# alibaba/EasyRec

Hardware: AMD Instinct MI355X
Metric: global examples/sec + emb HBM GB/s, DeepFM Criteo-shape b4096 @1/2/4/8 GPU (higher is better)
Workload: dtype f32; 1 GPU; DeepFM synthetic Criteo: deepfm_criteo.config (39 features: 26 hashed x 1000000 rows + 13 projected, D=16 deep + D=1 wide, batch 4096 per GPU, optimizer adam_optimizer (lazy dense decay, closed-form replay), ids zipf, hipGraph replay); timed steps cycle over 256 distinct device-generated batches after 1024 untimed pre-conditioning steps; global_batch=4096, parallelism=single GPU

## Files before the change

### easyrec_amd/csrc/er_embedding.hip

```cpp
#include <algorithm>
#include <cmath>
#include <cstring>
#include <vector>

#include "er_common.h"
#include "er_gemm_core.h"
#include "er_dense_tail.h"
#include "er_decay.h"
#include "er_grad_finish.h"

namespace er {

constexpr uint32_t kInvalidKey = 0xFFFFFFFFu;

__host__ __device__ __forceinline__ void lane_geom(int dim, int& V, int& G) {
  V = (dim % 4 == 0) ? 4 : 1;
  const int n = dim / V;
  G = 1;
  while (G < n) G <<= 1;
}

__device__ __forceinline__ int find_lookup(const int32_t* __restrict__ blk_start, int n, int bid) {
  int lo = 0, hi = n;
  while (hi - lo > 1) {
// ... 1457 lines not shown
  while (i + 1 < ma.n && static_cast<int>(blockIdx.x) >= ma.start[i + 1]) ++i;
  const RunArgs& a = ma.a[i];
  const int bid = blockIdx.x - ma.start[i];
  if (a.V == 4)
    tile_body<4>(bid, smem, a.skeys, a.svals, a.ent_gptr, a.ent_scale, a.n, a.dim, a.G, a.tab, ma.opt_kind, ma.hyper, a.ro,
                 a.tile_first, a.tile_last);
  else
    tile_body<1>(bid, smem, a.skeys, a.svals, a.ent_gptr, a.ent_scale, a.n, a.dim, a.G, a.tab, ma.opt_kind, ma.hyper, a.ro,
                 a.tile_first, a.tile_last);
}

__device__ __forceinline__ void tile_multi_block(int b, const RunMulti& ma, float* smem) {
  int i = 0;
  while (i + 1 < ma.n && b >= ma.start[i + 1]) ++i;
  const RunArgs& a = ma.a[i];
  const int bid = b - ma.start[i];
  if (a.V == 4)
    tile_body<4>(bid, smem, a.skeys, a.svals, a.ent_gptr, a.ent_scale, a.n, a.dim, a.G, a.tab, ma.opt_kind, ma.hyper, a.ro,
                 a.tile_first, a.tile_last);
  else
    tile_body<1>(bid, smem, a.skeys, a.svals, a.ent_gptr, a.ent_scale, a.n, a.dim, a.G, a.tab, ma.opt_kind, ma.hyper, a.ro,
                 a.tile_first, a.tile_last);
}

__global__ void __launch_bounds__(kBlock)
emb_reduce_local_wgrad_kernel(RunMulti ma, GroupedArgs ga, int n_gemm, int n_tile, LossTailArgs lt) {
  extern __shared__ __attribute__((aligned(16))) float smem[];
  const int bid = blockIdx.x;
  if (bid < n_gemm) {
    const GroupedCoords c = grouped_coords(ga, bid);
    if (c.split < 0) return;
    gemm_f32_block<false, false>(ga.p[c.p], c.tile, c.split, smem, c.plain);
    return;
  }
  if (bid - n_gemm < n_tile) tile_multi_block(bid - n_gemm, ma, smem);
  else loss_tail_body<kBlock>(lt, smem);
}

__device__ __forceinline__ void fix_block(int b, const RunMulti& ma) {
  int i = 0;
  while (i + 1 < ma.n && b >= ma.start[i + 1]) ++i;
  const RunArgs& a = ma.a[i];
  const int bid = b - ma.start[i];
  if (a.V == 4)
    fix_body<4>(bid, a.skeys, a.n, a.dim, a.G, a.T, a.n_tiles, a.tab, ma.opt_kind, ma.hyper, a.ro, a.tile_first,
                a.tile_last, a.aux);
  else
    fix_body<1>(bid, a.skeys, a.n, a.dim, a.G, a.T, a.n_tiles, a.tab, ma.opt_kind, ma.hyper, a.ro, a.tile_first,
                a.tile_last, a.aux);
}

__global__ void __launch_bounds__(kBlock)
emb_bwd_fix_multi_kernel(RunMulti ma) {
  fix_block(blockIdx.x, ma);
}

__global__ void __launch_bounds__(kBlock)
emb_bwd_fix_reduce_kernel(RunMulti ma, GroupedReduceArgs ra, int n_fix) {
  const int b = blockIdx.x;
  if (b < n_fix) fix_block(b, ma);
  else splitk_reduce_grouped_block<4>(ra, b - n_fix);
}

__global__ void __launch_bounds__(kBlock)
emb_bwd_fix_opt_kernel(RunMulti ma, GroupedReduceArgs ra, DenseOptArgs da, int n_fix) {
  __shared__ float red[4];
  const int b = blockIdx.x;
  if (b < n_fix) fix_block(b, ma);
  else dense_opt_block(da, ra, b - n_fix, red);
}

constexpr int kSegSortMax = 8192;
constexpr int kSegSortMin = 256;

template <typename C>
__device__ __forceinline__ void seg_cmpx(C& a, C& b, bool up) {
  const bool sw = (a > b) == up;
  const C lo = sw ? b : a, hi = sw ? a : b;
  a = lo;
  b = hi;
}

constexpr int kRadixBits = 5;
template <int E>
__device__ __forceinline__ void seg_radix_sort_narrow(uint32_t (&x)[E], uint32_t* buf , int P, int logP, uint32_t rel_max) {
  constexpr int NB = 1 << kRadixBits;
  constexpr int kMaxWaves = kSegSortMax / 8 / 64;
  __shared__ uint32_t cnt[NB * kMaxWaves];
  __shared__ uint32_t wtot[kMaxWaves];
  const int t = threadIdx.x, lane = t & 63, wave = t >> 6, nW = static_cast<int>(blockDim.x >> 6);
  const int n_cnt = NB * nW;
  uint32_t* A = buf;
  uint32_t* B = buf + P;
#pragma unroll
  for (int e = 0; e < E; ++e) A[t * E + e] = x[e];
  __syncthreads();
  const int key_bits = 32 - __clz(static_cast<int>(rel_max | 1u));
  const int chunk = wave * 64 * E;
  const unsigned long long lt_mask = (1ull << lane) - 1ull;
  uint32_t key[E];
#pragma unroll
  for (int e = 0; e < E; ++e) key[e] = A[chunk + e * 64 + lane];
  for (int shift = logP; shift < logP + key_bits; shift += kRadixBits) {
    if (t < n_cnt) cnt[t] = 0u;
    __syncthreads();
    uint32_t rank[E], slot[E];
#pragma unroll
    for (int e = 0; e < E; ++e) {
      const uint32_t d = (key[e] >> shift) & static_cast<uint32_t>(NB - 1);
      unsigned long long m = ~0ull;
#pragma unroll
      for (int b = 0; b < kRadixBits; ++b) {
        const bool bit = ((d >> b) & 1u) != 0u;
        const unsigned long long bal = __ballot(bit);
        m &= bit ? bal : ~bal;
      }
      const uint32_t lower = static_cast<uint32_t>(__popcll(m & lt_mask));
      const int sl = static_cast<int>(d) * nW + wave;
      const uint32_t prior = cnt[sl];
      rank[e] = prior + lower;
      slot[e] = static_cast<uint32_t>(sl);
      if (lower == 0u) cnt[sl] = prior + static_cast<uint32_t>(__popcll(m));
    }
    __syncthreads();
    uint32_t v = 0u, inc = 0u;
    if (t < n_cnt) v = cnt[t];
    inc = v;
#pragma unroll
    for (int dd = 1; dd < 64; dd <<= 1) {
      const uint32_t o = __shfl_up(inc, dd, 64);
      if (lane >= dd) inc += o;
    }
    if (lane == 63) wtot[wave] = inc;
    __syncthreads();
    uint32_t before = 0u;
    for (int w = 0; w < wave; ++w) before += wtot[w];
    if (t < n_cnt) cnt[t] = before + inc - v;
    __syncthreads();
#pragma unroll
    for (int e = 0; e < E; ++e) B[cnt[slot[e]] + rank[e]] = key[e];
    __syncthreads();
    uint32_t* T = A; A = B; B = T;
#pragma unroll
    for (int e = 0; e < E; ++e) key[e] = A[chunk + e * 64 + lane];
  }
#pragma unroll
  for (int e = 0; e < E; ++e) x[e] = A[t * E + e];
}

template <int E, bool HEADS, bool NARROW, bool INLINE>
__device__ __forceinline__ void seg_sort_body(int lk, const uint32_t* __restrict__ keys_in, const int64_t* __restrict__ ent_base,
                        const er_lookup_desc* __restrict__ descs, int P, Route rt, uint32_t* __restrict__ keys_out,
                        uint32_t* __restrict__ vals_out, uint32_t* __restrict__ flags_out,
                        uint32_t* __restrict__ hidx_out, uint32_t* __restrict__ seg_count, int skip_one_row,
                        unsigned long long* sk_raw, uint32_t* __restrict__ ukeys_seg = nullptr,
                        int64_t n_limit = INT64_MAX) {
  typedef typename std::conditional<NARROW, uint32_t, unsigned long long>::type C;
  C* sk = reinterpret_cast<C*>(sk_raw);
  constexpr int L = E == 8 ? 3 : (E == 4 ? 2 : 1);
  static_assert(E == 2 || E == 4 || E == 8, "E");
  const int t = threadIdx.x;
  const int i0 = t * E;
  const int64_t base = ent_base[lk];
  const int64_t end = ent_base[lk + 1] < n_limit ? ent_base[lk + 1] : n_limit;
  const int cnt = end > base ? static_cast<int>(end - base) : 0;
  const int logP = __ffs(P) - 1;
  const bool routed = rt.local_base != nullptr;
  const uint32_t stride = static_cast<uint32_t>(rt.shard_stride);
  uint32_t key_base = 0u, rows = 0u, srows = 1u;
  if (NARROW) {
    const er_lookup_desc& d = descs[lk];
    if (routed) {
      srows = static_cast<uint32_t>((d.rows + rt.world - 1) / rt.world);
      rows = srows * static_cast<uint32_t>(rt.world);
      key_base = static_cast<uint32_t>(rt.local_base[lk]);
    } else {
      rows = static_cast<uint32_t>(d.rows);
      key_base = static_cast<uint32_t>(d.key_base);
    }
  }
  auto key_of = [&](C c) -> uint32_t {
    if (NARROW) {
      const uint32_t rel = static_cast<uint32_t>(c >> logP);
      if (rel >= rows) return kInvalidKey;
      if (!routed) return rel + key_base;
      const uint32_t owner = rel / srows;
      return owner * stride + key_base + (rel - owner * srows);
    }
    return static_cast<uint32_t>(static_cast<unsigned long long>(c) >> 32);
  };
  C x[E];
#pragma unroll
  for (int e = 0; e < E; ++e) {
    const int i = i0 + e;
    if (i >= cnt) {
      x[e] = static_cast<C>(~0ull);
    } else if (INLINE) {
      const er_lookup_desc& d = descs[lk];
      const int64_t id = d.ids[i];
      bool ok = !(id < 0 || id >= d.rows);
      if (d.weights != nullptr && d.combiner != ER_COMBINER_SUM && !(d.weights[i] > 0.f)) ok = false;
      if (skip_one_row && d.rows == 1) ok = false;
      if (NARROW) {
        const uint32_t rel = ok ? static_cast<uint32_t>(id) : static_cast<uint32_t>(d.rows);
        x[e] = static_cast<C>((rel << logP) | static_cast<uint32_t>(i));
      } else {
        const uint32_t key = ok ? static_cast<uint32_t>(d.key_base + id) : kInvalidKey;
        x[e] = static_cast<C>((static_cast<unsigned long long>(key) << 32) | static_cast<unsigned>(base + i));
      }
    } else if (NARROW) {
      const uint32_t key = keys_in[base + i];
      uint32_t rel = rows;
      if (key != kInvalidKey) {
        if (routed) {
          const uint32_t owner = key / stride;
          rel = owner * srows + (key - owner * stride - key_base);
        } else {
          rel = key - key_base;
        }
      }
      x[e] = static_cast<C>((rel << logP) | static_cast<uint32_t>(i));
    } else {
      x[e] = static_cast<C>((static_cast<unsigned long long>(keys_in[base + i]) << 32) | static_cast<unsigned>(base + i));
    }
  }
  if constexpr (NARROW) {
    seg_radix_sort_narrow<E>(x, reinterpret_cast<uint32_t*>(sk_raw), P, logP, rows);
  } else
  for (int k = 2; k <= P; k <<= 1) {
    int j = k >> 1;
    bool in_lds = false;
    while (j >= 64 * E) {
      if (!in_lds) {
#pragma unroll
        for (int e = 0; e < E; ++e) sk[i0 + e] = x[e];
        __syncthreads();
      }
      const int b = __ffs(j) - 1, lb = b - L + 1;
      const int bs = ((t >> lb) << (b + 1)) | (t & ((1 << lb) - 1));
      const bool up = (bs & k) == 0;
      C y[E];
#pragma unroll
      for (int c = 0; c < E; ++c) y[c] = sk[bs + (c << lb)];
#pragma unroll
      for (int jj = E / 2; jj > 0; jj >>= 1)
#pragma unroll
        for (int c = 0; c < E; ++c)
          if ((c & jj) == 0) seg_cmpx(y[c], y[c | jj], up);
#pragma unroll
      for (int c = 0; c < E; ++c) sk[bs + (c << lb)] = y[c];
      __syncthreads();
      in_lds = true;
      j >>= L;
    }
    if (in_lds) {
#pragma unroll
      for (int e = 0; e < E; ++e) x[e] = sk[i0 + e];
    }
    if (j >= E) {
      const bool up = (i0 & k) == 0;
      for (; j >= E; j >>= 1) {
        const int lj = j / E;
        const bool keep_min = ((t & lj) == 0) == up;
#pragma unroll
        for (int e = 0; e < E; ++e) {
          const C o = __shfl_xor(x[e], lj);
          const C mn = x[e] < o ? x[e] : o, mx = x[e] < o ? o : x[e];
          x[e] = keep_min ? mn : mx;
        }
      }
    }
#pragma unroll
    for (int jj = E / 2; jj > 0; jj >>= 1) {
      if (jj <= j) {
#pragma unroll
        for (int e = 0; e < E; ++e)
          if ((e & jj) == 0) seg_cmpx(x[e], x[e | jj], ((i0 + e) & k) == 0);
      }
    }
  }
  uint32_t kk[E], ow[E];
#pragma unroll
  for (int e = 0; e < E; ++e) {
    kk[e] = key_of(x[e]);
    ow[e] = routed ? kk[e] / stride : 0u;
  }
#pragma unroll
  for (int e = 0; e < E; ++e) {
    const int i = i0 + e;
    if (i < cnt) {
      keys_out[base + i] = kk[e];
      vals_out[base + i] = NARROW ? static_cast<uint32_t>(base) + (static_cast<uint32_t>(x[e]) & static_cast<uint32_t>(P - 1))
                                  : static_cast<uint32_t>(static_cast<unsigned long long>(x[e]) & 0xFFFFFFFFu);
    }
  }
  if (HEADS) {
    __shared__ uint32_t wave_sum[kSegSortMax / 8 / 64];
    uint32_t* k32 = reinterpret_cast<uint32_t*>(sk_raw);
    __syncthreads();
#pragma unroll
    for (int e = 0; e < E; ++e) k32[i0 + e] = kk[e];
    __syncthreads();
    uint32_t prev = i0 > 0 ? k32[i0 - 1] : kInvalidKey;
    uint32_t f[E], c = 0;
#pragma unroll
    for (int e = 0; e < E; ++e) {
      const uint32_t key = kk[e];
      f[e] = (key != kInvalidKey && (i0 + e == 0 || prev != key)) ? 1u : 0u;
      c += f[e];
      prev = key;
    }
    const int lane = t & 63, wave = t >> 6, n_waves = blockDim.x >> 6;
    uint32_t inc = c;
#pragma unroll
    for (int d = 1; d < 64; d <<= 1) {
      const uint32_t o = __shfl_up(inc, d, 64);
      if (lane >= d) inc += o;
    }
    if (lane == 63) wave_sum[wave] = inc;
    __syncthreads();
    uint32_t before = 0, total = 0;
    for (int w = 0; w < n_waves; ++w) {
      const uint32_t ws = wave_sum[w];
      if (w < wave) before += ws;
      total += ws;
    }
    uint32_t run = before + inc - c;
#pragma unroll
    for (int e = 0; e < E; ++e) {
      const int i = i0 + e;
      if (i < cnt) {
        flags_out[base + i] = f[e];
        hidx_out[base + i] = run;
        if (ukeys_seg != nullptr && f[e]) ukeys_seg[base + run] = kk[e];
      }
      run += f[e];
    }
    if (!routed) {
      if (t == 0) seg_count[lk] = total;
    } else {
      __shared__ uint32_t owner_cnt[64];
      if (t < 64) owner_cnt[t] = 0u;
      __syncthreads();
#pragma unroll
      for (int e = 0; e < E; ++e)
        if (f[e]) atomicAdd(&owner_cnt[ow[e]], 1u);
      __syncthreads();
      if (t < 64) seg_count[lk * 64 + t] = owner_cnt[t];
    }
  }
}

template <int E, bool HEADS, bool NARROW>
__global__ void __launch_bounds__(kSegSortMax / 8)
emb_segment_sort_kernel(const uint32_t* __restrict__ keys_in, const int64_t* __restrict__ ent_base,
                        const er_lookup_desc* __restrict__ descs, int P, Route rt, uint32_t* __restrict__ keys_out,
                        uint32_t* __restrict__ vals_out, uint32_t* __restrict__ flags_out,
                        uint32_t* __restrict__ hidx_out, uint32_t* __restrict__ seg_count) {
  extern __shared__ __attribute__((aligned(16))) unsigned long long sk_raw[];
  seg_sort_body<E, HEADS, NARROW, false>(blockIdx.x, keys_in, ent_base, descs, P, rt, keys_out, vals_out, flags_out, hidx_out,
                                         seg_count, 0, sk_raw);
}

template <int E, bool NARROW>
__global__ void __launch_bounds__(kSegSortMax / 8)
emb_front_sort_kernel(const int64_t* __restrict__ ent_base, const er_lookup_desc* __restrict__ descs, int n_lookups, int P,
                      uint32_t* __restrict__ keys_out, uint32_t* __restrict__ vals_out, uint32_t* __restrict__ flags_out,
                      uint32_t* __restrict__ hidx_out, uint32_t* __restrict__ seg_count, int skip_one_row, DecayTabDev tabs,
                      const float* __restrict__ hist, const int64_t* __restrict__ counter, uint32_t* __restrict__ ukeys_seg) {
  extern __shared__ __attribute__((aligned(16))) unsigned long long sk_raw[];
  if (static_cast<int>(blockIdx.x) >= n_lookups) {
    const int k = (static_cast<int>(blockIdx.x) - n_lookups) * static_cast<int>(blockDim.x >> 6) + static_cast<int>(threadIdx.x >> 6) + 1;
    if (k > tabs.K) return;
    const int64_t s_end = *counter - 1;
    const float mine = decay_sum_wave(tabs, hist, s_end - 1 - k, k);
    const int lane = threadIdx.x & 63;
    float* A = tabs.A + static_cast<int64_t>(kDecayKMax) * kDecayLd;
    if (lane < kDecayLd) A[static_cast<int64_t>(k - 1) * kDecayLd + lane] = mine;
    return;
  }
  seg_sort_body<E, true, NARROW, true>(blockIdx.x, nullptr, ent_base, descs, P, Route{1, 0, nullptr}, keys_out, vals_out,
                                       flags_out, hidx_out, seg_count, skip_one_row, sk_raw, ukeys_seg);
}

template <int E, bool NARROW>
__global__ void __launch_bounds__(kSegSortMax / 8)
emb_front_fwd_kernel(const int64_t* __restrict__ ent_base, const er_lookup_desc* __restrict__ descs, int n_lookups, int P,
                     uint32_t* __restrict__ keys_out, uint32_t* __restrict__ vals_out, uint32_t* __restrict__ flags_out,
                     uint32_t* __restrict__ hidx_out, uint32_t* __restrict__ seg_count, int skip_one_row,
                     uint32_t* __restrict__ ukeys_seg, const er_lookup_desc* __restrict__ fwd_descs,
                     const int32_t* __restrict__ fwd_blk_start, int fwd_lookups, int fwd_blocks,
                     float* __restrict__ sumsq_partials, FwdLazy lz) {
  extern __shared__ __attribute__((aligned(16))) unsigned long long sk_raw[];
  if (static_cast<int>(blockIdx.x) < n_lookups) {
    seg_sort_body<E, true, NARROW, true>(blockIdx.x, nullptr, ent_base, descs, P, Route{1, 0, nullptr}, keys_out, vals_out,
                                         flags_out, hidx_out, seg_count, skip_one_row, sk_raw, ukeys_seg);
    return;
  }
  __shared__ float red[kSegSortMax / 8 / 64];
  const int per_wg = static_cast<int>(blockDim.x) / kBlock;
  const int vb = (static_cast<int>(blockIdx.x) - n_lookups) * per_wg + static_cast<int>(threadIdx.x) / kBlock;
  const int vt = static_cast<int>(threadIdx.x) % kBlock;
  float ss = 0.f;
  if (vb < fwd_blocks) ss = fwd_rows<true>(vb, vt, fwd_descs, fwd_blk_start, fwd_lookups, &lz);
  if (sumsq_partials) {
    ss = wave_sum(ss);
    const int wid = threadIdx.x >> 6;
    if ((threadIdx.x & 63) == 0) red[wid] = ss;
    __syncthreads();
    if (vt == 0 && vb < fwd_blocks) {
      const int w0 = (static_cast<int>(threadIdx.x) / kBlock) * 4;
      sumsq_partials[vb] = (red[w0] + red[w0 + 1]) + (red[w0 + 2] + red[w0 + 3]);
    }
  }
}

template <int E>
__global__ void __launch_bounds__(kSegSortMax / 8)
emb_chunk_sort_kernel(const uint32_t* __restrict__ keys_in, const int64_t* __restrict__ chunk_base, int P, int64_t n,
                      uint32_t* __restrict__ keys_out, uint32_t* __restrict__ vals_out) {
  extern __shared__ __attribute__((aligned(16))) unsigned long long sk_raw[];
  seg_sort_body<E, false, false, false>(blockIdx.x, keys_in, chunk_base, nullptr, P, Route{1, 0, nullptr}, keys_out, vals_out,
                                        nullptr, nullptr, nullptr, 0, sk_raw, nullptr, n);
}

constexpr int kChunkSortMax = 4096;
constexpr int kMergeVt = 8;
constexpr int kMergeTile = kBlock * kMergeVt;

__device__ __forceinline__ unsigned long long merge_comp(const uint32_t* __restrict__ k, const uint32_t* __restrict__ v, int64_t i) {
  return (static_cast<unsigned long long>(k[i]) << 32) | v[i];
}

template <typename GetA, typename GetB>
__device__ __forceinline__ int merge_path(int d, int na, int nb, GetA a_at, GetB b_at) {
  int lo = d > nb ? d - nb : 0, hi = d < na ? d : na;
  while (lo < hi) {
    const int mid = (lo + hi) >> 1;
    if (a_at(mid) < b_at(d - 1 - mid)) lo = mid + 1; else hi = mid;
  }
  return lo;
}

__global__ void __launch_bounds__(kBlock)
emb_merge_pass_kernel(const uint32_t* __restrict__ kin, const uint32_t* __restrict__ vin, int64_t n, int64_t run,
                      uint32_t* __restrict__ kout, uint32_t* __restrict__ vout) {
  __shared__ unsigned long long sm[kMergeTile];
  __shared__ int s_lo[2], s_hi[2];
  const int tid = threadIdx.x;
  const int64_t o0 = static_cast<int64_t>(blockIdx.x) * kMergeTile;
  const int64_t o1 = o0 + kMergeTile < n ? o0 + kMergeTile : n;
  const int64_t pair0 = (o0 / (2 * run)) * (2 * run);
  const int64_t a_beg = pair0;
  const int64_t a_end = a_beg + run < n ? a_beg + run : n;
  const int64_t b_end = a_end + run < n ? a_end + run : n;
  const int na = static_cast<int>(a_end - a_beg), nb = static_cast<int>(b_end - a_end);
  {
    constexpr int K = kBlock / 2;
    const int half = tid / K, t = tid % K;
    const int d = static_cast<int>((half == 0 ? o0 : o1) - pair0);
    if (t == 0) {
      s_lo[half] = d > nb ? d - nb : 0;
      s_hi[half] = d < na ? d : na;
    }
    __syncthreads();
    for (;;) {
      const int lo = s_lo[half], hi = s_hi[half];
      const int r = hi - lo;
      if (!__syncthreads_or(r > 0)) break;
      if (r > 0) {
        const int p = lo + static_cast<int>((static_cast<int64_t>(r) * (t + 1)) / (K + 1));
        const bool below = merge_comp(kin, vin, a_beg + p) < merge_comp(kin, vin, a_end + (d - 1 - p));
        if (below) atomicMax(&s_lo[half], p + 1); else atomicMin(&s_hi[half], p);
      }
      __syncthreads();
    }
  }
  const int a0 = s_lo[0], a1 = s_lo[1];
  const int b0 = static_cast<int>(o0 - pair0) - a0, b1 = static_cast<int>(o1 - pair0) - a1;
  const int ta = a1 - a0, tb = b1 - b0;
  const int total = ta + tb;
  {
    uint32_t kv[kMergeVt], vv[kMergeVt];
#pragma unroll
    for (int j = 0; j < kMergeVt; ++j) {
      int i = tid + j * kBlock;
      i = i < total ? i : total - 1;
      i = i < 0 ? 0 : i;
      const int64_t at = i < ta ? a_beg + a0 + i : a_end + b0 + (i - ta);
      kv[j] = kin[at];
      vv[j] = vin[at];
    }
#pragma unroll
    for (int j = 0; j < kMergeVt; ++j) {
      const int i = tid + j * kBlock;
      if (i < total) sm[i] = (static_cast<unsigned long long>(kv[j]) << 32) | vv[j];
    }
// ... 1462 lines not shown
  }
  g->ld = ld;
  g->ls_ld = last_step_ld;
  return 0;
}

static er::DecayAux decay_aux_for(const er_emb_group* g, int lag) {
  er::DecayAux a = g->aux;
  if (a.A != nullptr) a.A += static_cast<int64_t>(lag) * er::kDecayKMax * er::kDecayLd;
  return a;
}

static int launch_decay_tables(er_emb_group* const* groups, int n, int lag, hipStream_t s) {
  const er_decay_tables* done[er::kMaxMulti];
  int n_done = 0;
  for (int i = 0; i < n; ++i) {
    const er_decay_tables* t = groups[i] ? groups[i]->tabs : nullptr;
    bool seen = t == nullptr;
    for (int j = 0; j < n_done; ++j) seen = seen || done[j] == t;
    if (seen) continue;
    if (n_done < er::kMaxMulti) done[n_done++] = t;
    if (lag == 1 && t->lag1_built) {
      const_cast<er_decay_tables*>(t)->lag1_built = false;
      continue;
    }
    const int blocks = static_cast<int>(er::ceil_div(static_cast<int64_t>(t->dev.K) * er::kWave, er::kBlock));
    hipLaunchKernelGGL(er::decay_tables_kernel, dim3(blocks), dim3(er::kBlock), 0, s, t->dev, t->hist, t->counter, lag);
    ER_LAUNCH_CHECK();
  }
  return 0;
}

#define ER_ELIGIBLE(cond, ...)       \
  do {                               \
    if (!(cond)) {                   \
      er::set_error(__VA_ARGS__);    \
      return 3;                      \
    }                                \
  } while (0)

static int group_cap_shift(const er_emb_group* g) {
  const int64_t cap = g->h_descs[0].offsets ? g->h_descs[0].max_nnz : g->h_descs[0].n_rows;
  if (cap <= 0 || (cap & (cap - 1)) != 0) return -1;
  for (int i = 1; i < g->n; ++i)
    if ((g->h_descs[i].offsets ? g->h_descs[i].max_nnz : g->h_descs[i].n_rows) != cap) return -1;
  int sh = 0;
  while ((1LL << sh) < cap) ++sh;
  return sh;
}

static int front_collect_one_row(er_emb_group* g) {
  if (g->n_proj >= 0) return 0;
  std::vector<uint32_t> keys;
  std::vector<int32_t> idx;
  for (int i = 0; i < g->n; ++i)
    if (g->h_descs[i].rows == 1) {
      keys.push_back(static_cast<uint32_t>(g->h_descs[i].key_base));
      idx.push_back(i);
    }
  ER_REQUIRE(keys.size() <= 64, "er_emb_front: more than 64 one-row tables in a table group");
  g->n_proj = static_cast<int>(keys.size());
  if (g->n_proj > 0) {
    ER_CHECK_HIP(hipMalloc(&g->d_extra_keys, sizeof(uint32_t) * keys.size()));
    ER_CHECK_HIP(hipMalloc(&g->d_proj_lookup, sizeof(int32_t) * idx.size()));
    ER_CHECK_HIP(hipMalloc(&g->d_proj_partial, sizeof(float) * keys.size() * er::kProjParts * (g->dim + 1)));
    ER_CHECK_HIP(hipMalloc(&g->d_proj_ticket, sizeof(uint32_t) * keys.size()));
    ER_CHECK_HIP(hipMemcpy(g->d_extra_keys, keys.data(), sizeof(uint32_t) * keys.size(), hipMemcpyHostToDevice));
    ER_CHECK_HIP(hipMemcpy(g->d_proj_lookup, idx.data(), sizeof(int32_t) * idx.size(), hipMemcpyHostToDevice));
    ER_CHECK_HIP(hipMemset(g->d_proj_ticket, 0, sizeof(uint32_t) * keys.size()));
  }
  return 0;
}

struct FrontFwd {
  er_emb_plan* plan;
  float* sumsq;
  er::FwdLazy lz;
  bool launched;
};

static int fwd_lazy_prepare(er_emb_plan* p, er_emb_group* const* groups, int n, const er_opt_hyper* hyper, hipStream_t s,
                            er::FwdLazy* lz);

static int emb_front_impl(er_emb_group* const* groups, int n, int flags, const er_opt_hyper* hyper, hipStream_t s,
                          FrontFwd* ff) {
  ER_REQUIRE(groups && n >= 1 && n <= er::kMaxMulti, "er_emb_front: bad arguments (1 <= n <= %d)", er::kMaxMulti);
  const int skip_one_row = flags & ER_FRONT_SKIP_ONE_ROW;
  const bool defer = (flags & ER_FRONT_DEFER_CATCH_UP) != 0;
  for (int i = 0; i < n; ++i) {
    er_emb_group* g = groups[i];
    ER_REQUIRE(g, "er_emb_front: null group %d", i);
    ER_ELIGIBLE(g->d_local_base == nullptr && g->world == 1 && g->n_active < 0, "er_emb_front: group %d is routed / partly active", i);
    ER_ELIGIBLE(!g->has_ragged && g->seg_sort_pow2 > 0, "er_emb_front: group %d has ragged lookups or no per-lookup sort", i);
    ER_ELIGIBLE(!g->last_step || (g->tabs && g->G <= er::kWave), "er_emb_front: group %d replays its decay step by step", i);
    ER_ELIGIBLE(g->n <= er::kOwnMaxLookups, "er_emb_front: group %d has more than %d lookups", i, er::kOwnMaxLookups);
    if (g->last_step) ER_REQUIRE(hyper, "er_emb_front: the catch-up needs the step's er_opt_hyper");
    if (int rc = front_collect_one_row(g)) return rc;
  }
  bool tables_done = false;
  for (int i = 0; i < n; ++i)
    if (groups[i]->tabs && groups[i]->tabs->prologue_build) tables_done = true;
  if (tables_done)
    for (int i = 0; i < n; ++i)
      ER_REQUIRE(!groups[i]->tabs || groups[i]->tabs->prologue_build, "er_emb_front: the groups of one call must share their decay tables");
  int last_sort = -1;
  if (ff) {
    if (int rc = fwd_lazy_prepare(ff->plan, groups, n, hyper, s, &ff->lz)) return rc;
    for (int i = 0; i < n; ++i) {
      er_emb_group* g = groups[i];
      er_emb_group* l = g->leader;
      bool follows = false;
      if (l && emb_group_same_keys(g, l))
        for (int j = 0; j < i; ++j) follows = follows || groups[j] == l;
      if (!follows) last_sort = i;
    }
  }
  for (int i = 0; i < n; ++i) {
    er_emb_group* g = groups[i];
    er_emb_group* l = g->leader;
    bool follows = false;
    if (l && emb_group_same_keys(g, l))
      for (int j = 0; j < i; ++j) follows = follows || groups[j] == l;
    if (follows && l->front_epoch == l->sort_epoch && l->front_skip == (skip_one_row != 0)) {
      g->src = l;
      g->adopted_epoch = l->sort_epoch;
      g->sorted_valid = true;
      continue;
    }
    g->src = g;
    ++g->sort_epoch;
    const int P = g->seg_sort_pow2;
    const bool with_tables = g->tabs != nullptr && !tables_done;
    er::DecayTabDev tabs{};
    if (with_tables) tabs = g->tabs->dev;
    const int E = P > 4096 ? 8 : 4;
    const int threads = P / E;
    const int table_blocks = with_tables ? static_cast<int>(er::ceil_div(static_cast<int64_t>(tabs.K) * er::kWave, threads)) : 0;
    const size_t lds = sizeof(unsigned long long) * static_cast<size_t>(P);
    if (ff && i == last_sort && !with_tables && threads % er::kBlock == 0 && !ff->launched) {
      er_emb_plan* pl = ff->plan;
      const int per_wg = threads / er::kBlock;
      const int fwd_wgs = static_cast<int>(er::ceil_div(pl->n_blocks, per_wg));
#define ER_FRONT_FWD(EE, NRW)                                                                                             \
  hipLaunchKernelGGL((er::emb_front_fwd_kernel<EE, NRW>), dim3(g->n + fwd_wgs), dim3(threads), lds, s, g->d_ent_base,      \
                     g->d_descs, g->n, P, g->keys_out, g->vals_out, g->head_flags, g->head_index, g->seg_count,          \
                     skip_one_row ? 1 : 0, g->keys_in, pl->d_descs, pl->d_blk_start, pl->n, pl->n_blocks, ff->sumsq, ff->lz)
      if (E == 8) { if (g->seg_narrow) ER_FRONT_FWD(8, true); else ER_FRONT_FWD(8, false); }
      else { if (g->seg_narrow) ER_FRONT_FWD(4, true); else ER_FRONT_FWD(4, false); }
#undef ER_FRONT_FWD
      ER_LAUNCH_CHECK();
      ff->launched = true;
    } else {
#define ER_FRONT_SORT(EE, NRW)                                                                                           \
  hipLaunchKernelGGL((er::emb_front_sort_kernel<EE, NRW>), dim3(g->n + table_blocks), dim3(threads), lds, s, g->d_ent_base, \
                     g->d_descs, g->n, P, g->keys_out, g->vals_out, g->head_flags, g->head_index, g->seg_count,         \
                     skip_one_row ? 1 : 0, tabs, with_tables ? g->tabs->hist : nullptr, with_tables ? g->tabs->counter : nullptr, \
                     g->keys_in)
    if (E == 8) { if (g->seg_narrow) ER_FRONT_SORT(8, true); else ER_FRONT_SORT(8, false); }
    else { if (g->seg_narrow) ER_FRONT_SORT(4, true); else ER_FRONT_SORT(4, false); }
#undef ER_FRONT_SORT
    ER_LAUNCH_CHECK();
    }
    tables_done = tables_done || with_tables;
    g->heads_epoch = g->sort_epoch;
    g->front_epoch = g->sort_epoch;
    g->front_skip = skip_one_row != 0;
    g->sorted_valid = true;
  }
  for (int i = 0; i < n; ++i) groups[i]->front_deferred = defer && groups[i]->last_step != nullptr;
  if (defer) {
    for (int i = 0; i < n; ++i)
      if (groups[i]->last_step) ER_REQUIRE(tables_done, "er_emb_front: no sort leader carried the decay tables");
    return 0;
  }
  er::CatchHeadsMulti cm;
  cm.n = 0;
  cm.start[0] = 0;
  cm.hyper = hyper;
  const er_decay_tables* first_tabs = nullptr;
  for (int i = 0; i < n; ++i) {
    er_emb_group* g = groups[i];
    if (!g->last_step) continue;
    if (!first_tabs) first_tabs = g->tabs;
    ER_REQUIRE(g->tabs == first_tabs, "er_emb_front: the groups of one call must share their decay tables");
    const er_emb_group* src = g->src;
    er::CatchHeadsArgs& a = cm.a[cm.n];
    a.ukeys_seg = src->keys_in;
    a.seg_count = src->seg_count; a.ent_base = src->d_ent_base; a.n_lookups = src->n; a.n = group_entries(g);
    a.tab = tab_of(g);
    a.aux = decay_aux_for(g, 1);
    a.dim = g->dim; a.G = g->G; a.V = g->V;
    a.extra_keys = skip_one_row ? g->d_extra_keys : nullptr;
    a.n_extra = skip_one_row ? g->n_proj : 0;
    a.cap_shift = group_cap_shift(src);
    ER_REQUIRE(a.n_extra * g->G <= er::kBlock, "er_emb_front: group %d: %d one-row tables of %d lanes exceed a workgroup", i, a.n_extra, g->G);
    cm.start[cm.n + 1] = cm.start[cm.n] + static_cast<int>(er::ceil_div(a.n, er::kBlock / g->G)) + (a.n_extra > 0 ? 1 : 0);
    ++cm.n;
  }
  if (cm.n > 0) {
    ER_REQUIRE(tables_done, "er_emb_front: no sort leader carried the decay tables");
    hipLaunchKernelGGL(er::emb_catch_up_heads_kernel, dim3(cm.start[cm.n]), dim3(er::kBlock), 0, s, cm);
    ER_LAUNCH_CHECK();
  }
  return 0;
}

int er_emb_front(er_emb_group* const* groups, int n, int flags, const er_opt_hyper* hyper, er_stream_t stream) {
  return emb_front_impl(groups, n, flags, hyper, er::as_stream(stream), nullptr);
}

static unsigned long long* g_own_dbg = nullptr;
int er_debug_stamps(unsigned long long* p) { g_own_dbg = p; return 0; }

static int emb_bwd_fused_impl(er_emb_group* const* groups, int n, const er_grad_group* finish, int n_finish, int opt_kind,
                              const er_opt_hyper* hyper, const er_gemm_problem* wgrads, int n_wgrads, int wgrad_blocks,
                              const er_loss_tail_job* loss_tail, const er_dense_opt_job* dense_opt, er_stream_t stream) {
  ER_REQUIRE(groups && finish && hyper && n >= 1 && n <= er::kMaxMulti && n_finish >= 1 && n_finish <= er::kOwnMaxGG,
             "er_emb_bwd_fused: bad arguments (1 <= n <= %d groups, 1 <= n_finish <= %d)", er::kMaxMulti, er::kOwnMaxGG);
  ER_REQUIRE(opt_kind >= ER_OPT_SGD && opt_kind <= ER_OPT_ADAGRAD, "er_emb_bwd_fused: unknown optimizer %d", opt_kind);
  hipStream_t s = er::as_stream(stream);
  er::GroupedPlan plan;
  if (n_wgrads > 0) {
    ER_REQUIRE(wgrads && n_wgrads <= er::kMaxGroup, "er_emb_bwd_fused_wgrad: 1 <= n_wgrads <= %d", er::kMaxGroup);
    for (int i = 0; i < n_wgrads; ++i)
      ER_REQUIRE(!wgrads[i].col_stats && !wgrads[i].bn_partial,
                 "er_emb_bwd_fused_wgrad: problem %d: plain contractions only (no column statistics or BatchNorm epilogue)", i);
    if (int rc = er::plan_grouped(ER_GEMM_TN, wgrads, n_wgrads, false, &plan, wgrad_blocks)) return rc;
  }
  er::LossTailArgs lt;
  std::memset(&lt, 0, sizeof(lt));
  er::DenseOptArgs da;
  std::memset(&da, 0, sizeof(da));
  if (loss_tail || dense_opt) ER_REQUIRE(n_wgrads > 0, "er_emb_bwd_fused_tail: the riders need the weight gradients' launch (n_wgrads > 0)");
  if (loss_tail)
    if (int rc = er::make_loss_tail_args(loss_tail, &lt)) return rc;
  if (dense_opt) {
    if (int rc = er::make_dense_opt_args(dense_opt, &da)) return rc;
    for (int j = 0; j < plan.ra.n; ++j) {
      const er::ReduceItem& r = plan.ra.r[j];
      ER_REQUIRE(r.ldc == r.N && r.C >= da.grad && r.C + r.mn <= da.grad + da.n,
                 "er_emb_bwd_fused_tail: weight gradient %d is not a contiguous block of dense_opt->grad", j);
    }
    for (int i = 0; i < n_wgrads; ++i)
      ER_REQUIRE(wgrads[i].C, "er_emb_bwd_fused_tail: problem %d has no output", i);
  }
  er::OwnMulti ma;
  er::RunMulti fx;
  fx.n = 0;
  fx.start[0] = 0;
  fx.opt_kind = opt_kind;
  fx.hyper = hyper;
  ma.n = 0;
  ma.start[0] = 0;
  ma.proj_start[0] = 0;
  ma.opt_kind = opt_kind;
  ma.hyper = hyper;
  ma.n_gg = n_finish;
  ma.dbg = g_own_dbg;
  for (int k = 0; k < n_finish; ++k)
    ER_REQUIRE(finish[k].dout && finish[k].out && finish[k].n_terms >= 0 && finish[k].n_terms <= 4,
               "er_emb_bwd_fused: finish descriptor %d: bad arguments", k);
  hipStreamCaptureStatus cap = hipStreamCaptureStatusNone;
  (void)hipStreamIsCapturing(s, &cap);
  size_t lds = 0;
  for (int i = 0; i < n; ++i) {
    er_emb_group* g = groups[i];
    ER_REQUIRE(g, "er_emb_bwd_fused: null group %d", i);
    const er_emb_group* src = g->src;
    ER_REQUIRE(g->sorted_valid && src && src->front_epoch == src->sort_epoch,
               "er_emb_bwd_fused: call er_emb_front for this step first (group %d)", i);
    if (opt_kind == ER_OPT_ADAM || opt_kind == ER_OPT_LAZY_ADAM) ER_REQUIRE(g->m && g->v, "er_emb_bwd_fused: Adam needs m and v");
    if (opt_kind == ER_OPT_ADAGRAD) ER_REQUIRE(g->v, "er_emb_bwd_fused: Adagrad needs the accumulator in v");
    ER_REQUIRE(opt_kind != ER_OPT_ADAM || g->last_step, "er_emb_bwd_fused: ER_OPT_ADAM needs lazy dense decay (the sweep form: er_emb_bwd_update)");
    std::vector<er::OwnLookup> recs(g->n);
    for (int l = 0; l < g->n; ++l) {
      const er_lookup_desc& d = g->h_descs[l];
      int k_found = -1;
      for (int k = 0; k < n_finish; ++k)
        if (finish[k].dout == d.out && finish[k].ld == d.out_stride) k_found = k;
      ER_REQUIRE(k_found >= 0, "er_emb_bwd_fused: group %d lookup %d: no finish descriptor for its gradient buffer", i, l);
      const er_grad_group& fg = finish[k_found];
      ER_REQUIRE(d.n_rows <= fg.batch && d.out_col + d.dim <= fg.width,
                 "er_emb_bwd_fused: group %d lookup %d lies outside its gradient buffer", i, l);
      unsigned mask = 0;
      for (int t = 0; t < fg.n_terms; ++t) {
        const er_grad_term& q = fg.terms[t];
        const bool inside = d.out_col >= q.col0 && d.out_col + d.dim <= q.col0 + q.width;
        const bool outside = d.out_col + d.dim <= q.col0 || d.out_col >= q.col0 + q.width;
        ER_REQUIRE(inside || outside, "er_emb_bwd_fused: group %d lookup %d: a deferred term covers part of its columns", i, l);
        if (!inside) continue;
        if (q.kind == ER_GRAD_TERM_FM) {
          ER_REQUIRE(q.dim == d.dim && (d.out_col - q.col0) % q.dim == 0,
                     "er_emb_bwd_fused: group %d lookup %d is not one field of the FM term over its columns", i, l);
          mask |= 0x10u << t;
        }
// ... 992 lines not shown
```

Before: 14.01 million examples/s.

## Rework narrow segment radix sort with register histograms and wave-striped layout

The narrow radix sort now keeps keys in a wave-striped layout, builds per-wave digit histograms in lane registers via ballot masks and shuffles, and scans them with fewer barriers. It returns the sorted buffer directly and skips the initial LDS staging and final copy-back. Head-flag detection for narrow keys uses ballots over the sorted LDS buffer instead of a second LDS pass. It also batches the id, weight and key loads up front, adds an occupancy hint to launch bounds, and makes the block index wave-uniform. Optional timestamp probes are added but stay off unless a debug buffer is set. The main risk is correctness of the new rank and offset arithmetic and the bounds clamping.

```diff
diff --git a/easyrec_amd/csrc/er_embedding.hip b/easyrec_amd/csrc/er_embedding.hip
--- a/easyrec_amd/csrc/er_embedding.hip
+++ b/easyrec_amd/csrc/er_embedding.hip
@@ -1563,70 +1563,70 @@
 }
 
 constexpr int kRadixBits = 5;
+constexpr int64_t kFrontDbgOffset = 4096 * 16;
 template <int E>
-__device__ __forceinline__ void seg_radix_sort_narrow(uint32_t (&x)[E], uint32_t* buf , int P, int logP, uint32_t rel_max) {
+__device__ __forceinline__ const uint32_t* seg_radix_sort_narrow(uint32_t (&key)[E], uint32_t* buf , int P, int logP,
+                                                                 uint32_t rel_max, unsigned long long* dbg) {
   constexpr int NB = 1 << kRadixBits;
   constexpr int kMaxWaves = kSegSortMax / 8 / 64;
-  __shared__ uint32_t cnt[NB * kMaxWaves];
-  __shared__ uint32_t wtot[kMaxWaves];
+  static_assert(kRadixBits >= 1 && kRadixBits <= 6, "one histogram register per lane: at most 64 digits");
+  __shared__ uint32_t cnt[kMaxWaves * NB];
   const int t = threadIdx.x, lane = t & 63, wave = t >> 6, nW = static_cast<int>(blockDim.x >> 6);
-  const int n_cnt = NB * nW;
+  for (int i = nW * NB + t; i < kMaxWaves * NB; i += static_cast<int>(blockDim.x)) cnt[i] = 0u;
   uint32_t* A = buf;
   uint32_t* B = buf + P;
-#pragma unroll
-  for (int e = 0; e < E; ++e) A[t * E + e] = x[e];
-  __syncthreads();
   const int key_bits = 32 - __clz(static_cast<int>(rel_max | 1u));
   const int chunk = wave * 64 * E;
-  const unsigned long long lt_mask = (1ull << lane) - 1ull;
-  uint32_t key[E];
-#pragma unroll
-  for (int e = 0; e < E; ++e) key[e] = A[chunk + e * 64 + lane];
-  for (int shift = logP; shift < logP + key_bits; shift += kRadixBits) {
-    if (t < n_cnt) cnt[t] = 0u;
-    __syncthreads();
-    uint32_t rank[E], slot[E];
+  uint32_t inv[kRadixBits];
+#pragma unroll
+  for (int b = 0; b < kRadixBits; ++b) inv[b] = ((lane >> b) & 1) != 0 ? 0u : ~0u;
+  int pass = 0;
+  for (int shift = logP; shift < logP + key_bits; shift += kRadixBits, ++pass) {
+    uint32_t hist = 0u, rank[E], dig[E];
 #pragma unroll
     for (int e = 0; e < E; ++e) {
       const uint32_t d = (key[e] >> shift) & static_cast<uint32_t>(NB - 1);
-      unsigned long long m = ~0ull;
+      uint32_t lo = ~0u, hi = ~0u;
 #pragma unroll
       for (int b = 0; b < kRadixBits; ++b) {
-        const bool bit = ((d >> b) & 1u) != 0u;
-        const unsigned long long bal = __ballot(bit);
-        m &= bit ? bal : ~bal;
+        const unsigned long long bal = __ballot(((d >> b) & 1u) != 0u);
+        lo &= static_cast<uint32_t>(bal) ^ inv[b];
+        hi &= static_cast<uint32_t>(bal >> 32) ^ inv[b];
       }
-      const uint32_t lower = static_cast<uint32_t>(__popcll(m & lt_mask));
-      const int sl = static_cast<int>(d) * nW + wave;
-      const uint32_t prior = cnt[sl];
-      rank[e] = prior + lower;
-      slot[e] = static_cast<uint32_t>(sl);
-      if (lower == 0u) cnt[sl] = prior + static_cast<uint32_t>(__popcll(m));
-    }
+      const int src = static_cast<int>(d);
+      const uint32_t prior = static_cast<uint32_t>(__shfl(static_cast<int>(hist), src, 64));
+      const uint32_t own_lo = static_cast<uint32_t>(__shfl(static_cast<int>(lo), src, 64));
+      const uint32_t own_hi = static_cast<uint32_t>(__shfl(static_cast<int>(hi), src, 64));
+      rank[e] = prior + __builtin_amdgcn_mbcnt_hi(own_hi, __builtin_amdgcn_mbcnt_lo(own_lo, 0u));
+      dig[e] = d;
+      hist += static_cast<uint32_t>(__popc(lo)) + static_cast<uint32_t>(__popc(hi));
+    }
+    if (lane < NB) cnt[wave * NB + lane] = hist;
     __syncthreads();
-    uint32_t v = 0u, inc = 0u;
-    if (t < n_cnt) v = cnt[t];
-    inc = v;
-#pragma unroll
-    for (int dd = 1; dd < 64; dd <<= 1) {
+    uint32_t tot = 0u, pre = 0u;
+#pragma unroll
+    for (int w = 0; w < kMaxWaves; ++w) {
+      const uint32_t v = cnt[w * NB + (lane & (NB - 1))];
+      pre = w == wave ? tot : pre;
+      tot += v;
+    }
+    uint32_t inc = tot;
+#pragma unroll
+    for (int dd = 1; dd < NB; dd <<= 1) {
       const uint32_t o = __shfl_up(inc, dd, 64);
       if (lane >= dd) inc += o;
     }
-    if (lane == 63) wtot[wave] = inc;
-    __syncthreads();
-    uint32_t before = 0u;
-    for (int w = 0; w < wave; ++w) before += wtot[w];
-    if (t < n_cnt) cnt[t] = before + inc - v;
-    __syncthreads();
-#pragma unroll
-    for (int e = 0; e < E; ++e) B[cnt[slot[e]] + rank[e]] = key[e];
+    const uint32_t base = inc - tot + pre;
+#pragma unroll
+    for (int e = 0; e < E; ++e)
+      B[static_cast<uint32_t>(__shfl(static_cast<int>(base), static_cast<int>(dig[e]), 64)) + rank[e]] = key[e];
     __syncthreads();
     uint32_t* T = A; A = B; B = T;
 #pragma unroll
     for (int e = 0; e < E; ++e) key[e] = A[chunk + e * 64 + lane];
-  }
-#pragma unroll
-  for (int e = 0; e < E; ++e) x[e] = A[t * E + e];
+    if (dbg && t == 0 && pass < 8) dbg[8 + pass] = wall_clock64();
+  }
+  return A;
 }
 
 template <int E, bool HEADS, bool NARROW, bool INLINE>
@@ -1635,7 +1635,8 @@
                         uint32_t* __restrict__ vals_out, uint32_t* __restrict__ flags_out,
                         uint32_t* __restrict__ hidx_out, uint32_t* __restrict__ seg_count, int skip_one_row,
                         unsigned long long* sk_raw, uint32_t* __restrict__ ukeys_seg = nullptr,
-                        int64_t n_limit = INT64_MAX) {
+                        int64_t n_limit = INT64_MAX,
+                        unsigned long long* dbg = nullptr) {
   typedef typename std::conditional<NARROW, uint32_t, unsigned long long>::type C;
   C* sk = reinterpret_cast<C*>(sk_raw);
   constexpr int L = E == 8 ? 3 : (E == 4 ? 2 : 1);
@@ -1670,43 +1671,74 @@
     }
     return static_cast<uint32_t>(static_cast<unsigned long long>(c) >> 32);
   };
+  const int lane = t & 63, wave = t >> 6;
+  auto pos = [&](int e) -> int { return NARROW ? wave * 64 * E + e * 64 + lane : i0 + e; };
   C x[E];
-#pragma unroll
-  for (int e = 0; e < E; ++e) {
-    const int i = i0 + e;
-    if (i >= cnt) {
-      x[e] = static_cast<C>(~0ull);
-    } else if (INLINE) {
-      const er_lookup_desc& d = descs[lk];
-      const int64_t id = d.ids[i];
-      bool ok = !(id < 0 || id >= d.rows);
-      if (d.weights != nullptr && d.combiner != ER_COMBINER_SUM && !(d.weights[i] > 0.f)) ok = false;
+  if (INLINE) {
+    const er_lookup_desc& d = descs[lk];
+    const bool pruned = d.weights != nullptr && d.combiner != ER_COMBINER_SUM;
+    int64_t id[E];
+    float w[E];
+#pragma unroll
+    for (int e = 0; e < E; ++e) {
+      id[e] = 0;
+      w[e] = 1.f;
+    }
+    if (cnt > 0) {
+#pragma unroll
+      for (int e = 0; e < E; ++e) id[e] = d.ids[pos(e) < cnt ? pos(e) : cnt - 1];
+      if (pruned) {
+#pragma unroll
+        for (int e = 0; e < E; ++e) w[e] = d.weights[pos(e) < cnt ? pos(e) : cnt - 1];
+      }
+    }
+#pragma unroll
+    for (int e = 0; e < E; ++e) {
+      const int i = pos(e);
+      bool ok = !(id[e] < 0 || id[e] >= d.rows);
+      if (pruned && !(w[e] > 0.f)) ok = false;
       if (skip_one_row && d.rows == 1) ok = false;
       if (NARROW) {
-        const uint32_t rel = ok ? static_cast<uint32_t>(id) : static_cast<uint32_t>(d.rows);
+        const uint32_t rel = ok ? static_cast<uint32_t>(id[e]) : static_cast<uint32_t>(d.rows);
         x[e] = static_cast<C>((rel << logP) | static_cast<uint32_t>(i));
       } else {
-        const uint32_t key = ok ? static_cast<uint32_t>(d.key_base + id) : kInvalidKey;
+        const uint32_t key = ok ? static_cast<uint32_t>(d.key_base + id[e]) : kInvalidKey;
         x[e] = static_cast<C>((static_cast<unsigned long long>(key) << 32) | static_cast<unsigned>(base + i));
       }
-    } else if (NARROW) {
-      const uint32_t key = keys_in[base + i];
-      uint32_t rel = rows;
-      if (key != kInvalidKey) {
-        if (routed) {
-          const uint32_t owner = key / stride;
-          rel = owner * srows + (key - owner * stride - key_base);
-        } else {
-          rel = key - key_base;
+      if (i >= cnt) x[e] = static_cast<C>(~0ull);
+    }
+  } else {
+    uint32_t key[E];
+#pragma unroll
+    for (int e = 0; e < E; ++e) key[e] = kInvalidKey;
+    if (cnt > 0) {
+#pragma unroll
+      for (int e = 0; e < E; ++e) key[e] = keys_in[base + (pos(e) < cnt ? pos(e) : cnt - 1)];
+    }
+#pragma unroll
+    for (int e = 0; e < E; ++e) {
+      const int i = pos(e);
+      if (NARROW) {
+        uint32_t rel = rows;
+        if (key[e] != kInvalidKey) {
+          if (routed) {
+            const uint32_t owner = key[e] / stride;
+            rel = owner * srows + (key[e] - owner * stride - key_base);
+          } else {
+            rel = key[e] - key_base;
+          }
         }
+        x[e] = static_cast<C>((rel << logP) | static_cast<uint32_t>(i));
+      } else {
+        x[e] = static_cast<C>((static_cast<unsigned long long>(key[e]) << 32) | static_cast<unsigned>(base + i));
       }
-      x[e] = static_cast<C>((rel << logP) | static_cast<uint32_t>(i));
-    } else {
-      x[e] = static_cast<C>((static_cast<unsigned long long>(keys_in[base + i]) << 32) | static_cast<unsigned>(base + i));
-    }
-  }
+      if (i >= cnt) x[e] = static_cast<C>(~0ull);
+    }
+  }
+  if (dbg && t == 0) dbg[2] = wall_clock64();
+  const uint32_t* sorted = nullptr;
   if constexpr (NARROW) {
-    seg_radix_sort_narrow<E>(x, reinterpret_cast<uint32_t*>(sk_raw), P, logP, rows);
+    sorted = seg_radix_sort_narrow<E>(x, reinterpret_cast<uint32_t*>(sk_raw), P, logP, rows, dbg);
   } else
   for (int k = 2; k <= P; k <<= 1) {
     int j = k >> 1;
@@ -1766,57 +1798,94 @@
     kk[e] = key_of(x[e]);
     ow[e] = routed ? kk[e] / stride : 0u;
   }
+  if (dbg && t == 0) dbg[3] = wall_clock64();
 #pragma unroll
   for (int e = 0; e < E; ++e) {
-    const int i = i0 + e;
+    const int i = pos(e);
     if (i < cnt) {
       keys_out[base + i] = kk[e];
       vals_out[base + i] = NARROW ? static_cast<uint32_t>(base) + (static_cast<uint32_t>(x[e]) & static_cast<uint32_t>(P - 1))
                                   : static_cast<uint32_t>(static_cast<unsigned long long>(x[e]) & 0xFFFFFFFFu);
     }
   }
+  if (dbg && t == 0) dbg[4] = wall_clock64();
   if (HEADS) {
-    __shared__ uint32_t wave_sum[kSegSortMax / 8 / 64];
-    uint32_t* k32 = reinterpret_cast<uint32_t*>(sk_raw);
-    __syncthreads();
-#pragma unroll
-    for (int e = 0; e < E; ++e) k32[i0 + e] = kk[e];
-    __syncthreads();
-    uint32_t prev = i0 > 0 ? k32[i0 - 1] : kInvalidKey;
-    uint32_t f[E], c = 0;
+    constexpr int kMaxWaves = kSegSortMax / 8 / 64;
+    __shared__ __attribute__((aligned(16))) uint32_t wave_sum[kMaxWaves];
+    const int n_waves = blockDim.x >> 6;
+    uint32_t f[E], run[E], total = 0;
+    if constexpr (NARROW) {
+      const unsigned long long lt_mask = (1ull << lane) - 1ull;
+      uint32_t prev[E], heads = 0;
+#pragma unroll
+      for (int e = 0; e < E; ++e) prev[e] = sorted[pos(e) > 0 ? pos(e) - 1 : 0];
+#pragma unroll
+      for (int e = 0; e < E; ++e) {
+        const bool head = kk[e] != kInvalidKey && (pos(e) == 0 || (prev[e] >> logP) != (x[e] >> logP));
+        const unsigned long long bal = __ballot(head);
+        f[e] = head ? 1u : 0u;
+        run[e] = heads + static_cast<uint32_t>(__popcll(bal & lt_mask));
+        heads += static_cast<uint32_t>(__popcll(bal));
+      }
+      if (t < kMaxWaves && t >= n_waves) wave_sum[t] = 0u;
+      if (lane == 0) wave_sum[wave] = heads;
+      __syncthreads();
+      uint32_t before = 0;
+#pragma unroll
+      for (int q = 0; q < kMaxWaves / 4; ++q) {
+        const uint4 v = reinterpret_cast<const uint4*>(wave_sum)[q];
+        total += (v.x + v.y) + (v.z + v.w);
+        before += (q * 4 + 0 < wave ? v.x : 0u) + (q * 4 + 1 < wave ? v.y : 0u) + (q * 4 + 2 < wave ? v.z : 0u) +
+                  (q * 4 + 3 < wave ? v.w : 0u);
+      }
+#pragma unroll
+      for (int e = 0; e < E; ++e) run[e] += before;
+    } else {
+      uint32_t* k32 = reinterpret_cast<uint32_t*>(sk_raw);
+      __syncthreads();
+#pragma unroll
+      for (int e = 0; e < E; ++e) k32[i0 + e] = kk[e];
+      __syncthreads();
+      uint32_t prev = i0 > 0 ? k32[i0 - 1] : kInvalidKey;
+      uint32_t c = 0;
+#pragma unroll
+      for (int e = 0; e < E; ++e) {
+        const uint32_t key = kk[e];
+        f[e] = (key != kInvalidKey && (i0 + e == 0 || prev != key)) ? 1u : 0u;
+        c += f[e];
+        prev = key;
+      }
+      uint32_t inc = c;
+#pragma unroll
+      for (int d = 1; d < 64; d <<= 1) {
+        const uint32_t o = __shfl_up(inc, d, 64);
+        if (lane >= d) inc += o;
+      }
+      if (lane == 63) wave_sum[wave] = inc;
+      __syncthreads();
+      uint32_t before = 0;
+      for (int w = 0; w < n_waves; ++w) {
+        const uint32_t ws = wave_sum[w];
+        if (w < wave) before += ws;
+        total += ws;
+      }
+      uint32_t r = before + inc - c;
+#pragma unroll
+      for (int e = 0; e < E; ++e) {
+        run[e] = r;
+        r += f[e];
+      }
+    }
 #pragma unroll
     for (int e = 0; e < E; ++e) {
-      const uint32_t key = kk[e];
-      f[e] = (key != kInvalidKey && (i0 + e == 0 || prev != key)) ? 1u : 0u;
-      c += f[e];
-      prev = key;
-    }
-    const int lane = t & 63, wave = t >> 6, n_waves = blockDim.x >> 6;
-    uint32_t inc = c;
-#pragma unroll
-    for (int d = 1; d < 64; d <<= 1) {
-      const uint32_t o = __shfl_up(inc, d, 64);
-      if (lane >= d) inc += o;
-    }
-    if (lane == 63) wave_sum[wave] = inc;
-    __syncthreads();
-    uint32_t before = 0, total = 0;
-    for (int w = 0; w < n_waves; ++w) {
-      const uint32_t ws = wave_sum[w];
-      if (w < wave) before += ws;
-      total += ws;
-    }
-    uint32_t run = before + inc - c;
-#pragma unroll
-    for (int e = 0; e < E; ++e) {
-      const int i = i0 + e;
+      const int i = pos(e);
       if (i < cnt) {
         flags_out[base + i] = f[e];
-        hidx_out[base + i] = run;
-        if (ukeys_seg != nullptr && f[e]) ukeys_seg[base + run] = kk[e];
+        hidx_out[base + i] = run[e];
+        if (ukeys_seg != nullptr && f[e]) ukeys_seg[base + run[e]] = kk[e];
       }
-      run += f[e];
-    }
+    }
+    if (dbg && t == 0) dbg[5] = wall_clock64();
     if (!routed) {
       if (t == 0) seg_count[lk] = total;
     } else {
@@ -1865,22 +1934,26 @@
 }
 
 template <int E, bool NARROW>
-__global__ void __launch_bounds__(kSegSortMax / 8)
+__global__ void __launch_bounds__(kSegSortMax / 8, E == 4 ? 8 : 4)
 emb_front_fwd_kernel(const int64_t* __restrict__ ent_base, const er_lookup_desc* __restrict__ descs, int n_lookups, int P,
                      uint32_t* __restrict__ keys_out, uint32_t* __restrict__ vals_out, uint32_t* __restrict__ flags_out,
                      uint32_t* __restrict__ hidx_out, uint32_t* __restrict__ seg_count, int skip_one_row,
                      uint32_t* __restrict__ ukeys_seg, const er_lookup_desc* __restrict__ fwd_descs,
                      const int32_t* __restrict__ fwd_blk_start, int fwd_lookups, int fwd_blocks,
-                     float* __restrict__ sumsq_partials, FwdLazy lz) {
+                     float* __restrict__ sumsq_partials, FwdLazy lz, unsigned long long* dbg_all) {
   extern __shared__ __attribute__((aligned(16))) unsigned long long sk_raw[];
+  unsigned long long* dbg = dbg_all ? dbg_all + static_cast<int64_t>(blockIdx.x) * 16 : nullptr;
+  if (dbg && threadIdx.x == 0) dbg[0] = wall_clock64();
   if (static_cast<int>(blockIdx.x) < n_lookups) {
     seg_sort_body<E, true, NARROW, true>(blockIdx.x, nullptr, ent_base, descs, P, Route{1, 0, nullptr}, keys_out, vals_out,
-                                         flags_out, hidx_out, seg_count, skip_one_row, sk_raw, ukeys_seg);
+                                         flags_out, hidx_out, seg_count, skip_one_row, sk_raw, ukeys_seg, INT64_MAX, dbg);
+    if (dbg && threadIdx.x == 0) dbg[1] = wall_clock64();
     return;
   }
   __shared__ float red[kSegSortMax / 8 / 64];
   const int per_wg = static_cast<int>(blockDim.x) / kBlock;
-  const int vb = (static_cast<int>(blockIdx.x) - n_lookups) * per_wg + static_cast<int>(threadIdx.x) / kBlock;
+  const int vb = __builtin_amdgcn_readfirstlane((static_cast<int>(blockIdx.x) - n_lookups) * per_wg +
+                                                static_cast<int>(threadIdx.x) / kBlock);
   const int vt = static_cast<int>(threadIdx.x) % kBlock;
   float ss = 0.f;
   if (vb < fwd_blocks) ss = fwd_rows<true>(vb, vt, fwd_descs, fwd_blk_start, fwd_lookups, &lz);
@@ -1894,6 +1967,7 @@
       sumsq_partials[vb] = (red[w0] + red[w0 + 1]) + (red[w0 + 2] + red[w0 + 3]);
     }
   }
+  if (dbg && (threadIdx.x & 63) == 0) atomicMax(dbg + 1, static_cast<unsigned long long>(wall_clock64()));
 }
 
 template <int E>
@@ -3522,6 +3596,9 @@
 static int fwd_lazy_prepare(er_emb_plan* p, er_emb_group* const* groups, int n, const er_opt_hyper* hyper, hipStream_t s,
                             er::FwdLazy* lz);
 
+static unsigned long long* g_own_dbg = nullptr;
+int er_debug_stamps(unsigned long long* p) { g_own_dbg = p; return 0; }
+
 static int emb_front_impl(er_emb_group* const* groups, int n, int flags, const er_opt_hyper* hyper, hipStream_t s,
                           FrontFwd* ff) {
   ER_REQUIRE(groups && n >= 1 && n <= er::kMaxMulti, "er_emb_front: bad arguments (1 <= n <= %d)", er::kMaxMulti);
@@ -3581,10 +3658,12 @@
       er_emb_plan* pl = ff->plan;
       const int per_wg = threads / er::kBlock;
       const int fwd_wgs = static_cast<int>(er::ceil_div(pl->n_blocks, per_wg));
+      unsigned long long* fdbg = g_own_dbg && g->n + fwd_wgs <= 4096 ? g_own_dbg + er::kFrontDbgOffset : nullptr;
 #define ER_FRONT_FWD(EE, NRW)                                                                                             \
   hipLaunchKernelGGL((er::emb_front_fwd_kernel<EE, NRW>), dim3(g->n + fwd_wgs), dim3(threads), lds, s, g->d_ent_base,      \
                      g->d_descs, g->n, P, g->keys_out, g->vals_out, g->head_flags, g->head_index, g->seg_count,          \
-                     skip_one_row ? 1 : 0, g->keys_in, pl->d_descs, pl->d_blk_start, pl->n, pl->n_blocks, ff->sumsq, ff->lz)
+                     skip_one_row ? 1 : 0, g->keys_in, pl->d_descs, pl->d_blk_start, pl->n, pl->n_blocks, ff->sumsq, ff->lz, \
+                     fdbg)
       if (E == 8) { if (g->seg_narrow) ER_FRONT_FWD(8, true); else ER_FRONT_FWD(8, false); }
       else { if (g->seg_narrow) ER_FRONT_FWD(4, true); else ER_FRONT_FWD(4, false); }
 #undef ER_FRONT_FWD
@@ -3648,9 +3727,6 @@
 int er_emb_front(er_emb_group* const* groups, int n, int flags, const er_opt_hyper* hyper, er_stream_t stream) {
   return emb_front_impl(groups, n, flags, hyper, er::as_stream(stream), nullptr);
 }
-
-static unsigned long long* g_own_dbg = nullptr;
-int er_debug_stamps(unsigned long long* p) { g_own_dbg = p; return 0; }
 
 static int emb_bwd_fused_impl(er_emb_group* const* groups, int n, const er_grad_group* finish, int n_finish, int opt_kind,
                               const er_opt_hyper* hyper, const er_gemm_problem* wgrads, int n_wgrads, int wgrad_blocks,
```

Result: faster. 14.15 million examples/s (median of 6 runs) (+1.0%).
